# MorganGrundy/MosaicMagnifique

Hardware: NVIDIA B200
Metric: pixel-diffs/sec (higher is better)
Workload: dtype f32

## Files before the change

mosaicmagnifique_b200/csrc/diff_kernels.cu:

```cuda
#include <cuda_runtime.h>
#include <stdint.h>
#include <stdlib.h>

#include <algorithm>
#include <cub/device/device_scan.cuh>

#include "colour_math.cuh"
#include "kernels.h"

namespace mm {

__device__ __forceinline__ uint32_t smem_u32(const void *p) { return (uint32_t)__cvta_generic_to_shared(p); }

__device__ __forceinline__ void mbar_init(uint64_t *bar, uint32_t count)
{
    asm volatile("mbarrier.init.shared::cta.b64 [%0], %1;" ::"r"(smem_u32(bar)), "r"(count));
}
__device__ __forceinline__ void mbar_expect_tx(uint64_t *bar, uint32_t bytes)
{
    asm volatile("mbarrier.arrive.expect_tx.shared::cta.b64 _, [%0], %1;" ::"r"(smem_u32(bar)), "r"(bytes) : "memory");
}
__device__ __forceinline__ void mbar_arrive(uint64_t *bar)
{
    asm volatile("mbarrier.arrive.shared::cta.b64 _, [%0];" ::"r"(smem_u32(bar)) : "memory");
// ... 2 lines not shown
{
    asm volatile(
        "{\n"
        ".reg .pred p;\n"
        "WAIT_%=:\n"
        "mbarrier.try_wait.parity.shared::cta.b64 p, [%0], %1;\n"
        "@p bra DONE_%=;\n"
        "bra WAIT_%=;\n"
        "DONE_%=:\n"
        "}\n" ::"r"(smem_u32(bar)),
        "r"(parity)
        : "memory");
}
__device__ __forceinline__ void bulk_g2s(void *dst, const void *src, uint32_t bytes, uint64_t *bar)
{
    asm volatile("cp.async.bulk.shared::cluster.global.mbarrier::complete_tx::bytes [%0], [%1], %2, [%3];" ::"r"(
                     smem_u32(dst)),
                 "l"(src), "r"(bytes), "r"(smem_u32(bar))
                 : "memory");
}

#ifndef MM_PIXEL_UNROLL
#define MM_PIXEL_UNROLL 1
#endif
constexpr int kPixelUnroll = MM_PIXEL_UNROLL;
constexpr int kStages = MM_STAGES;
constexpr int kConsumerWarps = MM_TCB;
constexpr int kThreads = (kConsumerWarps + 1) * 32;
constexpr uint32_t kLibBlockBytes = MM_TNB * MM_KP * 16;
constexpr uint32_t kCellBlockBytes = MM_TCB * MM_KP * 20;
constexpr uint32_t kStageBytes = kLibBlockBytes + kCellBlockBytes;

template <int DIFF>
__device__ __forceinline__ void consume_ring(const unsigned char *smem, uint64_t *full_bar, uint64_t *empty_bar, int nk, int warp,
                                             int lane, float (&acc)[MM_TNB])
{
#pragma unroll
    for (int i = 0; i < MM_TNB; ++i)
        acc[i] = 0.0f;

    for (int k = 0; k < nk; ++k) {
        const int s = k % kStages;
        mbar_wait(&full_bar[s], (k / kStages) & 1);
        if (MM_STRESS_SKEW)
            __nanosleep((unsigned)((warp * 97 + k * 29 + blockIdx.x * 7) % 400));
        const float4 *lib_s = reinterpret_cast<const float4 *>(smem + (size_t)s * kStageBytes);
        const float4 *cell_s = reinterpret_cast<const float4 *>(smem + (size_t)s * kStageBytes + kLibBlockBytes) + warp * MM_KP;
        const float *w_s = reinterpret_cast<const float *>(smem + (size_t)s * kStageBytes + kLibBlockBytes + MM_TCB * MM_KP * 16) + warp * MM_KP;
#pragma unroll kPixelUnroll
        for (int j = 0; j < MM_KP / 32; ++j) {
            const int p = j * 32 + lane;
            const float4 c = cell_s[p];
            const float w = w_s[p];
            if (DIFF == MM_DIFF_CIEDE2000) {
#pragma unroll
                for (int i = 0; i < MM_TNB / 2; ++i) {
                    const float4 la = lib_s[(i * 2 + 0) * MM_KP + p];
                    const float4 lb = lib_s[(i * 2 + 1) * MM_KP + p];
                    const mm_f2 d = mm_ciede2000_stored_v<mm_f2>(c.x, c.y, c.z, c.w, mm_f2{la.x, la.y}, mm_f2{la.z, la.w},
                                                               mm_f2{lb.x, lb.y}, mm_f2{lb.z, lb.w});
                    const mm_f2 a2 = v_fma(mm_f2{w, w}, d, mm_f2{acc[2 * i], acc[2 * i + 1]});
                    acc[2 * i] = a2.x;
                    acc[2 * i + 1] = a2.y;
                }
            } else {
#pragma unroll
                for (int i = 0; i < MM_TNB; ++i) {
                    const float4 l = lib_s[i * MM_KP + p];
                    acc[i] = fmaf(w, mm_euclid(c.x, c.y, c.z, l.x, l.y, l.z), acc[i]);
                }
            }
        }
        __syncwarp();
        if (lane == 0)
            mbar_arrive(&empty_bar[s]);
    }
}

template <int DIFF>
__global__ void __launch_bounds__(kThreads, MM_MIN_CTAS)
diff_sum_kernel(const unsigned char *__restrict__ cells, const unsigned char *__restrict__ lib, float *__restrict__ D,
                unsigned long long *__restrict__ best_key, int n_chunks, int n_lib, int n_lib_pad, int n_cells,
                int n_cell_tiles, int n_lib_tiles, const int *__restrict__ cancel, unsigned long long *__restrict__ progress,
                int nk, int sb_a, int sb_b)
{
    extern __shared__ __align__(128) unsigned char smem[];
    __shared__ uint64_t full_bar[kStages];
    __shared__ uint64_t empty_bar[kStages];
    __shared__ int s_cancelled;

    const int warp = threadIdx.x >> 5, lane = threadIdx.x & 31;
    int cell_tile, lib_tile;
    {
        const unsigned id = blockIdx.x;
        const unsigned col_all = (unsigned)sb_a * (unsigned)n_lib_tiles;
        const unsigned cb = id / col_all;
        const unsigned r = id - cb * col_all;
        const int cw = min(sb_a, n_cell_tiles - (int)cb * sb_a);
        const unsigned band_ctas = (unsigned)cw * (unsigned)sb_b;
        const unsigned band = r / band_ctas;
        const unsigned r2 = r - band * band_ctas;
        cell_tile = (int)cb * sb_a + (int)(r2 % cw);
        lib_tile = (int)band * sb_b + (int)(r2 / cw);
    }

// ... 68 lines not shown
    if (e != cudaSuccess)
        return e;
    const unsigned grid = (unsigned)n_cell_tiles * (unsigned)n_lib_tiles;
    diff_sum_kernel<DIFF><<<grid, kThreads, smem, stream>>>((const unsigned char *)cells, (const unsigned char *)lib, D, best_key, n_chunks,
                                                            n_lib, n_lib_tiles * MM_TNB, n_cells, n_cell_tiles, n_lib_tiles, cancel,
                                                            progress, n_chunks, raster.sb_a, raster.sb_b);
    return cudaGetLastError();
}

cudaError_t launch_diff_sum(int diff_type, const void *cells, const void *lib, float *D, unsigned long long *best_key,
                            int n_cell_tiles, int n_lib_tiles, int n_chunks, int n_lib, int n_cells, cudaStream_t stream,
                            const int *cancel, unsigned long long *progress)
{
    if (n_cell_tiles <= 0 || n_lib_tiles <= 0 || n_chunks <= 0)
        return cudaSuccess;
    if (diff_type != MM_DIFF_CIEDE2000)
        return cudaErrorInvalidValue;
    auto env = [](const char *name) -> int {
        const char *v = getenv(name);
        return v ? atoi(v) : 0;
    };
    Raster r{std::min(kSuperTiles, n_cell_tiles), std::min(kSuperTiles, n_lib_tiles)};
    if (env("MM_SB_A") > 0)
        r.sb_a = std::min(env("MM_SB_A"), n_cell_tiles);
    if (env("MM_SB_B") > 0)
        r.sb_b = std::min(env("MM_SB_B"), n_lib_tiles);
    return launch<MM_DIFF_CIEDE2000>(cells, lib, D, best_key, n_cell_tiles, n_lib_tiles, n_chunks, n_lib, n_cells, stream, cancel, progress,
                                     r);
}


__global__ void __launch_bounds__(kThreads, MM_MIN_CTAS)
diff_rows_kernel(const unsigned char *__restrict__ cells, const unsigned char *__restrict__ lib, float *__restrict__ D, int n_chunks,
                 int nk, int n_lib_pad, int n_lib_tiles, RowList rows, const int *__restrict__ perm, const int *cancel,
                 unsigned long long *__restrict__ progress)
{
    extern __shared__ __align__(128) unsigned char smem[];
    __shared__ uint64_t full_bar[kStages];
    __shared__ uint64_t empty_bar[kStages];
    __shared__ int s_cancelled, s_cell[kConsumerWarps], s_lib_tile, s_n_rows;

    const int warp = threadIdx.x >> 5, lane = threadIdx.x & 31;
    if (threadIdx.x == 0) {
        const int cancelled = cancel ? load_cancel_flag(cancel) : 0;
        int lo = 0, hi = rows.n_buckets;
        while (hi - lo > 1) {
            const int mid = (lo + hi) >> 1;
            if (rows.groups[mid] <= (int)blockIdx.x)
                lo = mid;
            else
                hi = mid;
        }
        const int g = (int)blockIdx.x - rows.groups[lo];
        const int n_in = min(kConsumerWarps, rows.count[lo] - g * kConsumerWarps);
        const int *list = rows.cells + (size_t)lo * rows.col_cells + g * kConsumerWarps;
        for (int w = 0; w < kConsumerWarps; ++w)
            s_cell[w] = list[w < n_in ? w : 0];
        s_lib_tile = lo % n_lib_tiles;
        s_n_rows = n_in;
        for (int s = 0; s < kStages; ++s) {
            mbar_init(&full_bar[s], 1);
            mbar_init(&empty_bar[s], kConsumerWarps);
        }
        asm volatile("fence.mbarrier_init.release.cluster;" ::: "memory");
        s_cancelled = cancelled;
    }
    __syncthreads();
    if (s_cancelled)
        return;
    const int lib_tile = s_lib_tile;

    if (warp == kConsumerWarps) {
        if (lane == 0) {
            const unsigned char *lib_src = lib + (size_t)lib_tile * n_chunks * kLibBlockBytes;
            constexpr uint32_t kSlice = MM_KP * 16, kWSlice = MM_KP * 4;
            for (int k = 0; k < nk; ++k) {
                const int s = k % kStages;
                if (k >= kStages)
                    mbar_wait(&empty_bar[s], ((k / kStages) - 1) & 1);
                unsigned char *dst = smem + (size_t)s * kStageBytes;
                if (MM_STRESS_SKEW)
                    __nanosleep((unsigned)((k * 131 + blockIdx.x * 17) % 300));
                mbar_expect_tx(&full_bar[s], kLibBlockBytes + kConsumerWarps * (kSlice + kWSlice));
                bulk_g2s(dst, lib_src + (size_t)k * kLibBlockBytes, kLibBlockBytes, &full_bar[s]);
                for (int w = 0; w < kConsumerWarps; ++w) {
                    const int c = s_cell[w];
                    const unsigned char *blk = cells + ((size_t)(c / MM_TCB) * n_chunks + k) * kCellBlockBytes;
                    const int slot = c % MM_TCB;
                    bulk_g2s(dst + kLibBlockBytes + w * kSlice, blk + slot * kSlice, kSlice, &full_bar[s]);
                    bulk_g2s(dst + kLibBlockBytes + MM_TCB * kSlice + w * kWSlice, blk + MM_TCB * kSlice + slot * kWSlice, kWSlice,
                             &full_bar[s]);
                }
            }
        }
        return;
    }

    float acc[MM_TNB];
    consume_ring<MM_DIFF_CIEDE2000>(smem, full_bar, empty_bar, nk, warp, lane, acc);
#pragma unroll
    for (int i = 0; i < MM_TNB; ++i) {
        float v = acc[i];
#pragma unroll
        for (int o = 16; o > 0; o >>= 1)
            v += __shfl_xor_sync(0xffffffffu, v, o);
        acc[i] = v;
    }
    if (warp < s_n_rows && lane < MM_TNB) {
        float v = 0.0f;
#pragma unroll
        for (int i = 0; i < MM_TNB; ++i)
            v = (lane == i) ? acc[i] : v;
        float *d = D + (size_t)s_cell[warp] * n_lib_pad + perm[lib_tile * MM_TNB + lane];
        *d += v;
    }
    if (progress && threadIdx.x == 0)
        atomicAdd(progress, (unsigned long long)s_n_rows);
}

cudaError_t launch_diff_rows(const void *cells, const void *lib, float *D, int n_groups, int n_lib_tiles, int n_chunks, int k0, int nk,
                             RowList rows, const int *perm, cudaStream_t stream, const int *cancel, unsigned long long *progress)
{
    if (n_groups <= 0 || nk <= 0)
        return cudaSuccess;
    const size_t smem = (size_t)kStages * kStageBytes;
    cudaError_t e = cudaFuncSetAttribute(diff_rows_kernel, cudaFuncAttributeMaxDynamicSharedMemorySize, (int)smem);
    if (e != cudaSuccess)
        return e;
    diff_rows_kernel<<<(unsigned)n_groups, kThreads, smem, stream>>>(
        (const unsigned char *)cells + (size_t)k0 * kCellBlockBytes, (const unsigned char *)lib + (size_t)k0 * kLibBlockBytes, D, n_chunks, nk,
        n_lib_tiles * MM_TNB, n_lib_tiles, rows, perm, cancel, progress);
    return cudaGetLastError();
}

__global__ void __launch_bounds__(1024)
list_rows_kernel(float *__restrict__ D, int n_lib_pad, int n_lib, int n_rows, int n_lib_tiles, uint8_t *__restrict__ state, int want,
                 const float *__restrict__ T, const int *__restrict__ perm, int segs_left, RowList rows,
                 int *__restrict__ group_count, unsigned long long *__restrict__ listed, unsigned long long *__restrict__ progress)
{
    __shared__ int warp_sum[32];
    const int lib_tile = blockIdx.x, col = blockIdx.y;
    const int b = col * n_lib_tiles + lib_tile;
    const int cell = col * rows.col_cells + threadIdx.x;
    bool on = false;
    if (threadIdx.x < rows.col_cells && cell < n_rows) {
        uint8_t *st = state ? state + (size_t)cell * n_lib_tiles + lib_tile : nullptr;
        on = !st || *st == want;
        if (on && T) {
            const float t = T[cell];
            float *row = D + (size_t)cell * n_lib_pad;
            bool alive = false;
            for (int i = 0; i < MM_TNB; ++i) {
                const int j = perm[lib_tile * MM_TNB + i];
                alive = alive || (j < n_lib && row[j] <= t);
            }
            if (!alive) {
                for (int i = 0; i < MM_TNB; ++i)
                    row[perm[lib_tile * MM_TNB + i]] = __int_as_float(0x7f800000);
                *st = kRowDead;
                if (progress)
                    atomicAdd(progress, (unsigned long long)segs_left);
                on = false;
            }
        }
    }
    const int lane = threadIdx.x & 31, warp = threadIdx.x >> 5;
    const unsigned ballot = __ballot_sync(0xffffffffu, on);
    if (lane == 0)
        warp_sum[warp] = __popc(ballot);
    __syncthreads();
    int before = 0, total = 0;
    for (int w = 0; w < (int)(blockDim.x >> 5); ++w) {
        before += w < warp ? warp_sum[w] : 0;
        total += warp_sum[w];
    }
    if (on)
        rows.cells[(size_t)b * rows.col_cells + before + __popc(ballot & ((1u << lane) - 1u))] = cell;
    if (threadIdx.x == 0) {
        rows.count[b] = total;
        group_count[b] = (total + MM_TCB - 1) / MM_TCB;
        if (total)
            atomicAdd(listed, (unsigned long long)total);
    }
}

size_t list_rows_scratch_bytes(int n_buckets)
{
    size_t temp = 0;
    cub::DeviceScan::ExclusiveSum(nullptr, temp, (const int *)nullptr, (int *)nullptr, n_buckets + 1);
    return ((size_t)(n_buckets + 1) * sizeof(int) + 255 & ~(size_t)255) + temp;
}

cudaError_t launch_list_rows(float *D, int n_lib_pad, int n_lib, int n_rows, int n_lib_tiles, uint8_t *state, int want, const float *T,
                             const int *perm, int segs_left, RowList rows, void *scratch, size_t scratch_bytes,
                             unsigned long long *listed, unsigned long long *progress, cudaStream_t stream)
{
    const int n_cols = (n_rows + rows.col_cells - 1) / rows.col_cells;
    if (n_cols <= 0 || n_lib_tiles <= 0)
        return cudaSuccess;
    if (rows.col_cells > 1024 || rows.col_cells % 32 || rows.n_buckets != n_cols * n_lib_tiles)
        return cudaErrorInvalidValue;
    int *group_count = (int *)scratch;
    const size_t head = (size_t)(rows.n_buckets + 1) * sizeof(int) + 255 & ~(size_t)255;
    cudaError_t e = cudaMemsetAsync(group_count + rows.n_buckets, 0, sizeof(int), stream);
    if (e != cudaSuccess)
        return e;
    list_rows_kernel<<<dim3((unsigned)n_lib_tiles, (unsigned)n_cols), rows.col_cells, 0, stream>>>(
        D, n_lib_pad, n_lib, n_rows, n_lib_tiles, state, want, T, perm, segs_left, rows, group_count, listed, progress);
    if ((e = cudaGetLastError()) != cudaSuccess)
        return e;
    size_t temp = scratch_bytes - head;
    return cub::DeviceScan::ExclusiveSum((unsigned char *)scratch + head, temp, group_count, rows.groups, rows.n_buckets + 1, stream);
}

}
```

mosaicmagnifique_b200/csrc/generator.cu:

```cuda
#include <cuda_runtime.h>
#include <math.h>
#include <stdio.h>
#include <string.h>

#include <algorithm>
#include <atomic>
#include <chrono>
#include <string>
#include <thread>
#include <vector>

#include "../../include/mosaic_b200.h"
#include "host_model.h"
#include "kernels.h"

extern "C" const int16_t mm_lab_lut_s16[];

namespace {

using namespace mm;

struct Fail {
    int code;
    std::string msg;
// ... 27 lines not shown
    void release()
    {
        if (p)
            cudaFreeAsync(p, stream);
        p = nullptr;
        bytes = cap = 0;
    }
    template <typename T>
    T *as() const { return reinterpret_cast<T *>(p); }
    ~DevBuf() { release(); }
    DevBuf() = default;
    DevBuf(const DevBuf &) = delete;
    DevBuf &operator=(const DevBuf &) = delete;
    DevBuf(DevBuf &&o) noexcept : p(o.p), bytes(o.bytes), cap(o.cap), stream(o.stream)
    {
        o.p = nullptr;
        o.bytes = o.cap = 0;
    }
    DevBuf &operator=(DevBuf &&o) noexcept
    {
        if (this != &o) {
            release();
            p = o.p;
            bytes = o.bytes;
            cap = o.cap;
            stream = o.stream;
            o.p = nullptr;
            o.bytes = o.cap = 0;
        }
        return *this;
    }
};

constexpr int kPruneSegments = 8;
constexpr int kColumnCells = 256;

struct Workspace {
    DevBuf main_f32, main_var_u8, lib_small, lib_work, lib_half;
    DevBuf pix_list, masks4, descs, cells_packed, lib_packed, best_key;
    DevBuf grid, pos, next, prog, counts;
    DevBuf tab_start, tab_si, tab_alpha;
    DevBuf perm, inv_perm, order_scratch, row_cells, row_count, row_groups, list_scratch, row_state, listed, prune_score, prune_idx,
        threshold;
    DevBuf prefix_score, prefix_idx;
};

struct StepPlan {
    int rows = 0, cols = 0;
    int S = 0, ds = 0, k = 1;
    int n_active = 0, n_chunks = 0;
    std::vector<int> cell_pos;
    std::vector<int> next_x;
    std::vector<int> row_first;
    int64_t cell_begin = 0, cell_end = 0;
    int64_t per_rank = 0;
    double pixel_diffs = 0, pixel_diffs_nominal = 0;
};

struct StepOut {
    DevBuf D;
    DevBuf cand;
    DevBuf margins;
    bool have_D = false, have_margins = false;
    int cand_k = 0;
};

struct Handles {
    cudaStream_t stream = nullptr;
    cudaStream_t poll_stream = nullptr;
    int *h_cancel = nullptr;
    int *d_cancel = nullptr;
    unsigned long long *h_progress = nullptr;

    Handles() = default;
    Handles(const Handles &) = delete;
    Handles &operator=(const Handles &) = delete;
// ... 655 lines not shown
    w.n_rows_local = (int)(w.n_local * V);
    w.n_cell_tiles = (w.n_rows_local + tg.tcb - 1) / tg.tcb;
    w.n_rows_pad = w.n_cell_tiles * tg.tcb;
    d.descs.alloc(std::max<size_t>(descs.size(), 1) * sizeof(CellDesc), st);
    CU(cudaMemcpyAsync(d.descs.p, descs.data(), descs.size() * sizeof(CellDesc), cudaMemcpyHostToDevice, st));
    tm.h2d_bytes += (double)(descs.size() * sizeof(CellDesc));
    d.cells_packed.alloc((size_t)std::max(w.n_cell_tiles, 1) * p.n_chunks * tg.cell_block, st);
    AreaTab cell_tab{nullptr, nullptr, nullptr};
    if (p.k == 0)
        cell_tab = upload_area_table(g, p.S, p.ds, tm);
    CU(launch_extract_cells(d.main_f32.as<float>(), g->img_rows, g->img_cols, d.descs.as<CellDesc>(), w.n_rows_local, p.S, p.ds, p.k,
                            cell_tab, d.masks4.as<uint8_t>(), d.pix_list.as<int>(), p.n_active, p.n_chunks, d.cells_packed.p, r.layout,
                            st));
    tm.kernel_launches++;
}

void plan_step(const G *g, const Run &r, size_t s, StepWork &w)
{
    const StepPlan &p = g->plans[s];
    const int64_t N = r.N;
    w.need_D = !r.fused_argmin || g->keep_D;
    const int64_t rr = g->repeat_range;
    const int64_t n_win = 2 * rr * rr + 2 * rr;
    const int64_t n_excl = r.capped ? r.O * exhausted_bound(g, s) : 0;
    w.k_need = r.candidates_only ? ((r.penalise || r.capped) ? std::min<int64_t>(N, r.O * n_win + n_excl + 1) : 1)
                                 : std::min<int64_t>(N, r.O * n_win + n_excl + 1 + (g->report_margins ? 1 : 0));
    w.via_topk = r.candidates_only || ((r.penalise || r.capped) && w.k_need * 4 <= N);
    w.M = (int)std::min<int64_t>(N, w.k_need + w.k_need / 4 + 8);
    w.prune = r.row_passes && w.via_topk && r.V == 1 && !g->keep_D && w.k_need * 4 <= N && w.M <= 4096 && w.n_rows_local > 0;
    w.n_segs = 1;
    w.seg_chunks = p.n_chunks;
    if (r.row_passes) {
        const char *ev = getenv("MM_SPLITK");
        const int want = ev && atoi(ev) > 0 ? atoi(ev) : kPruneSegments;
        w.seg_chunks = (p.n_chunks + std::min(want, p.n_chunks) - 1) / std::min(want, p.n_chunks);
        w.n_segs = (p.n_chunks + w.seg_chunks - 1) / w.seg_chunks;
        if (const char *ea = getenv("MM_SB_A"))
            w.col_cells = std::max(32, std::min(1024, atoi(ea) * MM_TCB / 32 * 32));
    }
    w.prog_total = r.row_passes ? (unsigned long long)std::max(w.n_rows_local, 1) * r.n_lib_tiles * w.n_segs
                                : (unsigned long long)std::max(w.n_cell_tiles, 1) * r.n_lib_tiles;
}

double difference_sums(G *g, const Run &r, size_t s, const StepWork &w, Progress &prog, mosaic_timings &tm)
{
    cudaStream_t st = g->stream;
    const StepPlan &p = g->plans[s];
    Workspace &d = g->ws;
    StepOut &o = g->out[s];
    DevBuf &D = o.D;
    if (w.need_D) {
        D.alloc((size_t)std::max(w.n_rows_pad, 1) * r.n_lib_pad * sizeof(float), st);
        o.have_D = true;
    }
    if (r.fused_argmin) {
        d.best_key.alloc((size_t)std::max(w.n_rows_pad, 1) * sizeof(unsigned long long), st);
        CU(launch_fill_u64(d.best_key.as<unsigned long long>(), (size_t)std::max(w.n_rows_pad, 1), ~0ull, st));
        tm.kernel_launches++;
    }
    prog.start_step(s, w.prog_total);
    if (!r.row_passes || w.n_rows_local == 0) {
        float *Dp = w.need_D ? D.as<float>() : nullptr;
        unsigned long long *keys = r.fused_argmin ? d.best_key.as<unsigned long long>() : nullptr;
        if (r.layout == kLayoutCiede)
            CU(launch_diff_sum(MM_DIFF_CIEDE2000, d.cells_packed.p, d.lib_packed.p, Dp, keys, w.n_cell_tiles, r.n_lib_tiles, p.n_chunks,
                               (int)r.N, w.n_rows_local, st, g->d_cancel, prog.d_done));
        else
            CU(launch_diff_euclid(d.cells_packed.p, d.lib_packed.p, Dp, keys, w.n_cell_tiles, r.n_lib_tiles, p.n_chunks, (int)r.N,
                                  w.n_rows_local, st, g->d_cancel, prog.d_done));
        tm.kernel_launches += w.n_cell_tiles > 0;
        return 1.0;
    }

    CU(cudaMemsetAsync(D.p, 0, D.bytes, st));
    const int n_cols = (w.n_rows_local + w.col_cells - 1) / w.col_cells;
    RowList rows{nullptr, nullptr, nullptr, n_cols * r.n_lib_tiles, w.col_cells};
    d.row_cells.alloc((size_t)rows.n_buckets * w.col_cells * sizeof(int), st);
    d.row_count.alloc((size_t)rows.n_buckets * sizeof(int), st);
    d.row_groups.alloc((size_t)(rows.n_buckets + 1) * sizeof(int), st);
    d.list_scratch.alloc(list_rows_scratch_bytes(rows.n_buckets), st);
    d.listed.alloc(sizeof(unsigned long long), st);
    rows.cells = d.row_cells.as<int>();
    rows.count = d.row_count.as<int>();
    rows.groups = d.row_groups.as<int>();
    const int *perm = d.perm.as<int>();
    uint8_t *state = nullptr;
    if (w.prune) {
        d.row_state.alloc((size_t)w.n_rows_local * r.n_lib_tiles, st);
        CU(cudaMemsetAsync(d.row_state.p, kRowActive, d.row_state.bytes, st));
        state = d.row_state.as<uint8_t>();
    }
    double units = 0;
    int n_groups = 0;
    auto list = [&](uint8_t *st8, int want, const float *T, int segs_left) {
        CU(cudaMemsetAsync(d.listed.p, 0, sizeof(unsigned long long), st));
        CU(launch_list_rows(D.as<float>(), r.n_lib_pad, (int)r.N, w.n_rows_local, r.n_lib_tiles, st8, want, T, perm, segs_left, rows,
                            d.list_scratch.p, d.list_scratch.bytes, d.listed.as<unsigned long long>(), prog.d_done, st));
        CU(cudaMemcpyAsync(g->h_progress + 1, rows.groups + rows.n_buckets, sizeof(int), cudaMemcpyDeviceToHost, st));
        CU(cudaMemcpyAsync(g->h_progress + 2, d.listed.p, sizeof(unsigned long long), cudaMemcpyDeviceToHost, st));
        tm.kernel_launches += 2;
        prog.wait();
        n_groups = (int)*reinterpret_cast<const int *>(g->h_progress + 1);
        return (double)g->h_progress[2];
    };
    auto pass = [&](int seg, double n_listed) {
        const int k0 = seg * w.seg_chunks, nk = std::min(p.n_chunks, k0 + w.seg_chunks) - k0;
        CU(launch_diff_rows(d.cells_packed.p, d.lib_packed.p, D.as<float>(), n_groups, r.n_lib_tiles, p.n_chunks, k0, nk, rows, perm, st,
                            g->d_cancel, prog.d_done));
        tm.kernel_launches += n_groups > 0;
        units += n_listed * nk;
    };
    double n_listed = list(nullptr, kRowActive, nullptr, 0);
    if (!w.prune) {
        for (int seg = 0; seg < w.n_segs; ++seg)
            pass(seg, n_listed);
    } else {
        pass(0, n_listed);
        d.prune_score.alloc((size_t)w.n_rows_local * w.M * sizeof(float), st);
        d.prune_idx.alloc((size_t)w.n_rows_local * w.M * sizeof(int), st);
        d.threshold.alloc((size_t)w.n_rows_local * sizeof(float), st);
        CU(launch_topk(D.as<float>(), r.n_lib_pad, (int)r.N, w.n_rows_local, w.M, d.prune_score.as<float>(), d.prune_idx.as<int>(), st));
        CU(launch_prune_threshold(D.as<float>(), r.n_lib_pad, d.prune_idx.as<int>(), w.n_rows_local, w.M, (int)w.k_need,
                                  d.inv_perm.as<int>(), r.n_lib_tiles, state, nullptr, true, st));
        tm.kernel_launches += 2;
        if (w.n_segs > 1) {
            n_listed = list(state, kRowComplete, nullptr, 0);
            for (int seg = 1; seg < w.n_segs; ++seg)
                pass(seg, n_listed);
        }
        CU(launch_prune_threshold(D.as<float>(), r.n_lib_pad, d.prune_idx.as<int>(), w.n_rows_local, w.M, (int)w.k_need,
                                  d.inv_perm.as<int>(), r.n_lib_tiles, state, d.threshold.as<float>(), false, st));
        tm.kernel_launches++;
        for (int seg = 1; seg < w.n_segs; ++seg) {
            n_listed = list(state, kRowActive, d.threshold.as<float>(), w.n_segs - seg);
            pass(seg, n_listed);
        }
    }
    return units / ((double)w.n_rows_local * r.n_lib_tiles * p.n_chunks);
}

struct Candidates {
    const float *scores = nullptr;
    const int *idx = nullptr;
    int M = 0, M_stride = 0;
    const float *pscores = nullptr;
    const int *pidx = nullptr;
    int k0 = 0, p_stride = 0;
    long long rows_per_block = 0, block_stride = 0;
};

template <typename Source>
void select_step(G *g, size_t s, const unsigned long long *keys, Source &&candidates, int max_uses, bool restart_used, float *margins,
                 PhaseClock *launch_clock, mosaic_timings &tm)
{
    const StepPlan &p = g->plans[s];
    GridStep &gs = g->grid[s];
    Workspace &w = g->ws;
    cudaStream_t st = g->stream;
    const int n_all = (int)p.cell_pos.size();
    w.grid.alloc(gs.v.size() * sizeof(long long), st);
    CU(cudaMemcpyAsync(w.grid.p, gs.v.data(), gs.v.size() * sizeof(long long), cudaMemcpyHostToDevice, st));
    w.pos.alloc(std::max<size_t>(p.cell_pos.size(), 1) * sizeof(int), st);
    CU(cudaMemcpyAsync(w.pos.p, p.cell_pos.data(), p.cell_pos.size() * sizeof(int), cudaMemcpyHostToDevice, st));
    tm.h2d_bytes += (double)(gs.v.size() * sizeof(long long) + p.cell_pos.size() * sizeof(int));
    if (keys) {
        CU(launch_keys_to_grid(keys, w.pos.as<int>(), w.grid.as<long long>(), n_all, nullptr, st));
    } else {
        w.next.alloc(std::max<size_t>(p.next_x.size(), 1) * sizeof(int), st);
        CU(cudaMemcpyAsync(w.next.p, p.next_x.data(), p.next_x.size() * sizeof(int), cudaMemcpyHostToDevice, st));
        w.prog.alloc((size_t)p.rows * sizeof(int), st);
        CU(cudaMemcpyAsync(w.prog.p, p.row_first.data(), (size_t)p.rows * sizeof(int), cudaMemcpyHostToDevice, st));
// ... 124 lines not shown
    if (!g->d_lut.p) {
        const std::vector<int16_t> lut4 = expand_lab_lut(mm_lab_lut_s16);
        g->d_lut.alloc(lut4.size() * sizeof(int16_t), st);
        CU(cudaMemcpyAsync(g->d_lut.p, lut4.data(), g->d_lut.bytes, cudaMemcpyHostToDevice, st));
        CU(cudaStreamSynchronize(st));
        tm.h2d_bytes += (double)g->d_lut.bytes;
    }

    clock.begin(kPre);
    main_to_working_space(g, r, tm);
    const LibSource lib = prepare_library(g, r, tm);
    clock.end();

    if (g->out.size() != n_steps) {
        g->out.clear();
        g->out.resize(n_steps);
    }
    for (StepOut &o : g->out) {
        o.have_D = o.have_margins = false;
        o.cand_k = 0;
    }
    if (candidates_only) {
        g->cand_max_uses = g->max_uses;
        g->cap_last_step = -1;
    }
    if (r.row_passes) {
        g->ws.perm.alloc((size_t)r.n_lib_pad * sizeof(int), st);
        g->ws.inv_perm.alloc((size_t)r.n_lib_pad * sizeof(int), st);
        g->ws.order_scratch.alloc(library_order_scratch_bytes(r.N), st);
        CU(launch_library_order(lib.oriented, g->lib_stored_size, r.N, r.n_lib_pad, g->ws.perm.as<int>(), g->ws.inv_perm.as<int>(),
                                g->ws.order_scratch.p, g->ws.order_scratch.bytes, st));
        tm.kernel_launches += 3;
    }
    Progress prog(g);
    for (size_t s = 0; s < n_steps; ++s) {
        prog.check_cancel();
        StepWork w;
        clock.begin(kPre);
        prepare_step(g, r, lib, s, w, tm);
        clock.end();
        plan_step(g, r, s, w);

        clock.begin(kDiff);
        const double evaluated = difference_sums(g, r, s, w, prog, tm);
        tm.evaluated_pixel_diffs += g->plans[s].pixel_diffs * evaluated;
        clock.end();
        if (g->progress_fn)
            prog.wait();

        clock.begin(kSel);
        select_phase(g, r, s, w, tm);
        clock.end();
        prog.end_step();
    }
    prog.finish();
    tm.preprocess_ms = clock.sum(kPre);
    tm.diff_ms = clock.sum(kDiff);
    tm.select_ms = clock.sum(kSel);
    tm.total_ms = std::chrono::duration<double, std::milli>(std::chrono::steady_clock::now() - t_host0).count();
}

}


extern "C" {

const char *mosaic_version(void) { return "mosaicmagnifique_b200 0.1 (sm_100a)"; }

int mosaic_create(int device, mosaic_generator **out)
{
    if (!out)
        return MOSAIC_ERR_INVALID_ARGUMENT;
    *out = nullptr;
    int count = 0;
    if (cudaGetDeviceCount(&count) != cudaSuccess || device < 0 || device >= count) {
        cudaGetLastError();
        return MOSAIC_ERR_CUDA;
    }
    mosaic_generator *g = new (std::nothrow) mosaic_generator();
    if (!g)
        return MOSAIC_ERR_OUT_OF_MEMORY;
    g->device = device;
    if (cudaSetDevice(device) != cudaSuccess || cudaStreamCreateWithFlags(&g->stream, cudaStreamNonBlocking) != cudaSuccess ||
        cudaStreamCreateWithFlags(&g->poll_stream, cudaStreamNonBlocking) != cudaSuccess ||
        cudaHostAlloc((void **)&g->h_cancel, sizeof(int), cudaHostAllocDefault) != cudaSuccess ||
        cudaMalloc((void **)&g->d_cancel, 256) != cudaSuccess || cudaMemset(g->d_cancel, 0, 256) != cudaSuccess ||
        cudaHostAlloc((void **)&g->h_progress, 4 * sizeof(unsigned long long), cudaHostAllocDefault) != cudaSuccess) {
        mosaic_destroy(g);
// ... 775 lines not shown
```

mosaicmagnifique_b200/csrc/kernels.h:

```cpp
#pragma once
#include <cuda_runtime.h>
#include <stdint.h>

#include <vector>

#define MM_DIFF_RGB_EUCLIDEAN 0
#define MM_DIFF_CIE76 1
#define MM_DIFF_CIEDE2000 2
#define MM_DIFF_EUCLID 0

#define MM_TCB 8
#define MM_TNB 8
#ifndef MM_KP
#define MM_KP 128
#endif
#ifndef MM_STAGES
#define MM_STAGES 3
#endif
#ifndef MM_ESTAGES
#define MM_ESTAGES 3
#endif
#ifndef MM_STRESS_SKEW
#define MM_STRESS_SKEW 0
#endif
// ... 22 lines not shown
{
    const unsigned band_ctas = (unsigned)n_ct * kSuperTiles;
    const unsigned band = id / band_ctas;
    const unsigned r = id - band * band_ctas;
    const int band_h = min(kSuperTiles, n_lt - (int)band * kSuperTiles);
    const unsigned col_ctas = (unsigned)kSuperTiles * band_h;
    const unsigned cb = r / col_ctas;
    const unsigned r2 = r - cb * col_ctas;
    const int cw = min(kSuperTiles, n_ct - (int)cb * kSuperTiles);
    cell_tile = (int)cb * kSuperTiles + (int)(r2 % cw);
    lib_tile = (int)band * kSuperTiles + (int)(r2 / cw);
}
#endif

enum PackLayout { kLayoutCiede = 0, kLayoutEuclid = 1 };
struct TileGeom {
    int tcb, tnb, kp;
    size_t cell_block, lib_block;
};
inline TileGeom tile_geom(PackLayout l)
{
    return l == kLayoutEuclid ? TileGeom{MM_ETC, MM_ETN, MM_EKP, (size_t)MM_EKP * 4 * MM_ETC * 4, (size_t)MM_EKP * 3 * MM_ETN * 4}
                              : TileGeom{MM_TCB, MM_TNB, MM_KP, (size_t)MM_TCB * MM_KP * 20, (size_t)MM_TNB * MM_KP * 16};
}

cudaError_t launch_diff_euclid(const void *cells, const void *lib, float *D, unsigned long long *best_key, int n_cell_tiles,
                               int n_lib_tiles, int n_chunks, int n_lib, int n_cells, cudaStream_t stream,
                               const int *cancel = nullptr, unsigned long long *progress = nullptr);

cudaError_t launch_diff_sum(int diff_type, const void *cells, const void *lib, float *D, unsigned long long *best_key,
                            int n_cell_tiles, int n_lib_tiles, int n_chunks, int n_lib, int n_cells, cudaStream_t stream,
                            const int *cancel = nullptr, unsigned long long *progress = nullptr);

struct RowList {
    int *cells;
    int *count;
    int *groups;
    int n_buckets, col_cells;
};
enum : uint8_t { kRowActive = 0, kRowComplete = 1, kRowDead = 2 };
cudaError_t launch_diff_rows(const void *cells, const void *lib, float *D, int n_groups, int n_lib_tiles, int n_chunks, int k0, int nk,
                             RowList rows, const int *perm, cudaStream_t stream, const int *cancel = nullptr,
                             unsigned long long *progress = nullptr);
size_t list_rows_scratch_bytes(int n_buckets);
cudaError_t launch_list_rows(float *D, int n_lib_pad, int n_lib, int n_rows, int n_lib_tiles, uint8_t *state, int want, const float *T,
                             const int *perm, int segs_left, RowList rows, void *scratch, size_t scratch_bytes,
                             unsigned long long *listed, unsigned long long *progress, cudaStream_t stream);

cudaError_t launch_to_working_space(const uint8_t *bgr, size_t row_stride, int rows, int cols, float *out, bool is_lab,
                                    const short4 *lab_lut, const int *c8, cudaStream_t stream);
constexpr size_t kLabLutEntries = 33 * 33 * 33;
inline std::vector<int16_t> expand_lab_lut(const int16_t *lut3)
{
    std::vector<int16_t> out(kLabLutEntries * 4, 0);
    for (size_t i = 0; i < kLabLutEntries; ++i)
        for (int c = 0; c < 3; ++c)
            out[i * 4 + c] = lut3[i * 3 + c];
    return out;
}
cudaError_t launch_hue_rotate(const uint8_t *in, uint8_t *out, int rows, int cols, float rot, cudaStream_t stream);
cudaError_t launch_area_u8(const uint8_t *src, uint8_t *dst, int64_t n, int src_size, int k, cudaStream_t stream);
cudaError_t launch_orient_library(const uint8_t *src, uint8_t *dst, int64_t n, int S, int flips, cudaStream_t stream);
cudaError_t launch_area_f32(const float *src, float *dst, int64_t n, int src_size, int k, cudaStream_t stream);
struct AreaTab {
    const int *start;
    const int *si;
    const float *alpha;
};
cudaError_t launch_area_general_u8(const uint8_t *src, uint8_t *dst, int64_t n, int src_size, int dst_size, AreaTab tab,
                                   cudaStream_t stream);
cudaError_t launch_area_general_f32(const float *src, float *dst, int64_t n, int src_size, int dst_size, AreaTab tab,
                                    cudaStream_t stream);
struct CubicTab {
    const int *idx;
    const int16_t *coef;
};
cudaError_t launch_cubic_u8(const uint8_t *src, int sh, int sw, int cn, uint8_t *dst, int dh, int dw, CubicTab xt, CubicTab yt,
                            cudaStream_t stream);
cudaError_t launch_pack_library(const float *lib, void *packed, int64_t n, int P, const int *pix_list, int n_active,
                                int n_chunks, int n_lib_tiles, PackLayout layout, cudaStream_t stream, const int *perm = nullptr);
// ... 71 lines not shown
```

Measured before the change: 437.4 billion.

## Make row-pass kernel persistent with atomic group queue and no host sync

Converts the diff_rows kernel from one CTA per group into a persistent grid sized by occupancy. The producer warp pulls group descriptors from a global atomic counter and signals consumers through a shared ring, so groups flow through the pipeline without refilling per CTA. It also removes the per-pass host round-trip that read group counts, computing group descriptors on device and accumulating evaluated units on device, read once at the end. Segment sizing changes to fixed chunk counts. The exchange is an extra describe kernel and an atomic per group, plus more complex termination and cancellation logic.

```diff
diff --git a/mosaicmagnifique_b200/csrc/diff_kernels.cu b/mosaicmagnifique_b200/csrc/diff_kernels.cu
--- a/mosaicmagnifique_b200/csrc/diff_kernels.cu
+++ b/mosaicmagnifique_b200/csrc/diff_kernels.cu
@@ -58,6 +58,38 @@
 constexpr uint32_t kStageBytes = kLibBlockBytes + kCellBlockBytes;
 
 template <int DIFF>
+__device__ __forceinline__ void consume_stage(const unsigned char *smem, int s, int warp, int lane, float (&acc)[MM_TNB])
+{
+    const float4 *lib_s = reinterpret_cast<const float4 *>(smem + (size_t)s * kStageBytes);
+    const float4 *cell_s = reinterpret_cast<const float4 *>(smem + (size_t)s * kStageBytes + kLibBlockBytes) + warp * MM_KP;
+    const float *w_s = reinterpret_cast<const float *>(smem + (size_t)s * kStageBytes + kLibBlockBytes + MM_TCB * MM_KP * 16) + warp * MM_KP;
+#pragma unroll kPixelUnroll
+    for (int j = 0; j < MM_KP / 32; ++j) {
+        const int p = j * 32 + lane;
+        const float4 c = cell_s[p];
+        const float w = w_s[p];
+        if (DIFF == MM_DIFF_CIEDE2000) {
+#pragma unroll
+            for (int i = 0; i < MM_TNB / 2; ++i) {
+                const float4 la = lib_s[(i * 2 + 0) * MM_KP + p];
+                const float4 lb = lib_s[(i * 2 + 1) * MM_KP + p];
+                const mm_f2 d = mm_ciede2000_stored_v<mm_f2>(c.x, c.y, c.z, c.w, mm_f2{la.x, la.y}, mm_f2{la.z, la.w},
+                                                           mm_f2{lb.x, lb.y}, mm_f2{lb.z, lb.w});
+                const mm_f2 a2 = v_fma(mm_f2{w, w}, d, mm_f2{acc[2 * i], acc[2 * i + 1]});
+                acc[2 * i] = a2.x;
+                acc[2 * i + 1] = a2.y;
+            }
+        } else {
+#pragma unroll
+            for (int i = 0; i < MM_TNB; ++i) {
+                const float4 l = lib_s[i * MM_KP + p];
+                acc[i] = fmaf(w, mm_euclid(c.x, c.y, c.z, l.x, l.y, l.z), acc[i]);
+            }
+        }
+    }
+}
+
+template <int DIFF>
 __device__ __forceinline__ void consume_ring(const unsigned char *smem, uint64_t *full_bar, uint64_t *empty_bar, int nk, int warp,
                                              int lane, float (&acc)[MM_TNB])
 {
@@ -70,33 +102,7 @@
         mbar_wait(&full_bar[s], (k / kStages) & 1);
         if (MM_STRESS_SKEW)
             __nanosleep((unsigned)((warp * 97 + k * 29 + blockIdx.x * 7) % 400));
-        const float4 *lib_s = reinterpret_cast<const float4 *>(smem + (size_t)s * kStageBytes);
-        const float4 *cell_s = reinterpret_cast<const float4 *>(smem + (size_t)s * kStageBytes + kLibBlockBytes) + warp * MM_KP;
-        const float *w_s = reinterpret_cast<const float *>(smem + (size_t)s * kStageBytes + kLibBlockBytes + MM_TCB * MM_KP * 16) + warp * MM_KP;
-#pragma unroll kPixelUnroll
-        for (int j = 0; j < MM_KP / 32; ++j) {
-            const int p = j * 32 + lane;
-            const float4 c = cell_s[p];
-            const float w = w_s[p];
-            if (DIFF == MM_DIFF_CIEDE2000) {
-#pragma unroll
-                for (int i = 0; i < MM_TNB / 2; ++i) {
-                    const float4 la = lib_s[(i * 2 + 0) * MM_KP + p];
-                    const float4 lb = lib_s[(i * 2 + 1) * MM_KP + p];
-                    const mm_f2 d = mm_ciede2000_stored_v<mm_f2>(c.x, c.y, c.z, c.w, mm_f2{la.x, la.y}, mm_f2{la.z, la.w},
-                                                               mm_f2{lb.x, lb.y}, mm_f2{lb.z, lb.w});
-                    const mm_f2 a2 = v_fma(mm_f2{w, w}, d, mm_f2{acc[2 * i], acc[2 * i + 1]});
-                    acc[2 * i] = a2.x;
-                    acc[2 * i + 1] = a2.y;
-                }
-            } else {
-#pragma unroll
-                for (int i = 0; i < MM_TNB; ++i) {
-                    const float4 l = lib_s[i * MM_KP + p];
-                    acc[i] = fmaf(w, mm_euclid(c.x, c.y, c.z, l.x, l.y, l.z), acc[i]);
-                }
-            }
-        }
+        consume_stage<DIFF>(smem, s, warp, lane, acc);
         __syncwarp();
         if (lane == 0)
             mbar_arrive(&empty_bar[s]);
@@ -231,32 +237,17 @@
 
 __global__ void __launch_bounds__(kThreads, MM_MIN_CTAS)
 diff_rows_kernel(const unsigned char *__restrict__ cells, const unsigned char *__restrict__ lib, float *__restrict__ D, int n_chunks,
-                 int nk, int n_lib_pad, int n_lib_tiles, RowList rows, const int *__restrict__ perm, const int *cancel,
+                 int nk, int n_lib_pad, RowList rows, const int *__restrict__ perm, const int *cancel,
                  unsigned long long *__restrict__ progress)
 {
     extern __shared__ __align__(128) unsigned char smem[];
     __shared__ uint64_t full_bar[kStages];
     __shared__ uint64_t empty_bar[kStages];
-    __shared__ int s_cancelled, s_cell[kConsumerWarps], s_lib_tile, s_n_rows;
+    __shared__ int s_cancelled, s_group[kStages];
 
     const int warp = threadIdx.x >> 5, lane = threadIdx.x & 31;
     if (threadIdx.x == 0) {
         const int cancelled = cancel ? load_cancel_flag(cancel) : 0;
-        int lo = 0, hi = rows.n_buckets;
-        while (hi - lo > 1) {
-            const int mid = (lo + hi) >> 1;
-            if (rows.groups[mid] <= (int)blockIdx.x)
-                lo = mid;
-            else
-                hi = mid;
-        }
-        const int g = (int)blockIdx.x - rows.groups[lo];
-        const int n_in = min(kConsumerWarps, rows.count[lo] - g * kConsumerWarps);
-        const int *list = rows.cells + (size_t)lo * rows.col_cells + g * kConsumerWarps;
-        for (int w = 0; w < kConsumerWarps; ++w)
-            s_cell[w] = list[w < n_in ? w : 0];
-        s_lib_tile = lo % n_lib_tiles;
-        s_n_rows = n_in;
         for (int s = 0; s < kStages; ++s) {
             mbar_init(&full_bar[s], 1);
             mbar_init(&empty_bar[s], kConsumerWarps);
@@ -267,75 +258,121 @@
     __syncthreads();
     if (s_cancelled)
         return;
-    const int lib_tile = s_lib_tile;
 
     if (warp == kConsumerWarps) {
         if (lane == 0) {
-            const unsigned char *lib_src = lib + (size_t)lib_tile * n_chunks * kLibBlockBytes;
             constexpr uint32_t kSlice = MM_KP * 16, kWSlice = MM_KP * 4;
-            for (int k = 0; k < nk; ++k) {
-                const int s = k % kStages;
-                if (k >= kStages)
-                    mbar_wait(&empty_bar[s], ((k / kStages) - 1) & 1);
-                unsigned char *dst = smem + (size_t)s * kStageBytes;
-                if (MM_STRESS_SKEW)
-                    __nanosleep((unsigned)((k * 131 + blockIdx.x * 17) % 300));
-                mbar_expect_tx(&full_bar[s], kLibBlockBytes + kConsumerWarps * (kSlice + kWSlice));
-                bulk_g2s(dst, lib_src + (size_t)k * kLibBlockBytes, kLibBlockBytes, &full_bar[s]);
-                for (int w = 0; w < kConsumerWarps; ++w) {
-                    const int c = s_cell[w];
-                    const unsigned char *blk = cells + ((size_t)(c / MM_TCB) * n_chunks + k) * kCellBlockBytes;
-                    const int slot = c % MM_TCB;
-                    bulk_g2s(dst + kLibBlockBytes + w * kSlice, blk + slot * kSlice, kSlice, &full_bar[s]);
-                    bulk_g2s(dst + kLibBlockBytes + MM_TCB * kSlice + w * kWSlice, blk + MM_TCB * kSlice + slot * kWSlice, kWSlice,
-                             &full_bar[s]);
+            const int n_groups = rows.groups[rows.n_buckets];
+            for (int t = 0;;) {
+                const int cancelled = t > 0 && cancel ? load_cancel_flag(cancel) : 0;
+                const int g = atomicAdd(rows.next, 1);
+                const bool stop = g >= n_groups || cancelled;
+                int s = t % kStages;
+                if (t >= kStages)
+                    mbar_wait(&empty_bar[s], ((t / kStages) - 1) & 1);
+                *(volatile int *)&s_group[s] = stop ? -1 : g;
+                if (stop) {
+                    mbar_arrive(&full_bar[s]);
+                    return;
                 }
+                const GroupDesc &gd = rows.desc[g];
+                int cell[kConsumerWarps];
+#pragma unroll
+                for (int w = 0; w < kConsumerWarps; ++w)
+                    cell[w] = gd.cell[w];
+                const unsigned char *lib_src = lib + (size_t)gd.lib_tile * n_chunks * kLibBlockBytes;
+                for (int k = 0; k < nk; ++k, ++t, s = t % kStages) {
+                    if (k > 0 && t >= kStages)
+                        mbar_wait(&empty_bar[s], ((t / kStages) - 1) & 1);
+                    unsigned char *dst = smem + (size_t)s * kStageBytes;
+                    if (MM_STRESS_SKEW)
+                        __nanosleep((unsigned)((t * 131 + blockIdx.x * 17) % 300));
+                    mbar_expect_tx(&full_bar[s], kLibBlockBytes + kConsumerWarps * (kSlice + kWSlice));
+                    bulk_g2s(dst, lib_src + (size_t)k * kLibBlockBytes, kLibBlockBytes, &full_bar[s]);
+#pragma unroll
+                    for (int w = 0; w < kConsumerWarps; ++w) {
+                        const int c = cell[w];
+                        const unsigned char *blk = cells + ((size_t)(c / MM_TCB) * n_chunks + k) * kCellBlockBytes;
+                        const int slot = c % MM_TCB;
+                        bulk_g2s(dst + kLibBlockBytes + w * kSlice, blk + slot * kSlice, kSlice, &full_bar[s]);
+                        bulk_g2s(dst + kLibBlockBytes + MM_TCB * kSlice + w * kWSlice, blk + MM_TCB * kSlice + slot * kWSlice, kWSlice,
+                                 &full_bar[s]);
+                    }
+                }
             }
         }
         return;
     }
 
     float acc[MM_TNB];
-    consume_ring<MM_DIFF_CIEDE2000>(smem, full_bar, empty_bar, nk, warp, lane, acc);
-#pragma unroll
-    for (int i = 0; i < MM_TNB; ++i) {
-        float v = acc[i];
-#pragma unroll
-        for (int o = 16; o > 0; o >>= 1)
-            v += __shfl_xor_sync(0xffffffffu, v, o);
-        acc[i] = v;
-    }
-    if (warp < s_n_rows && lane < MM_TNB) {
-        float v = 0.0f;
+#pragma unroll
+    for (int i = 0; i < MM_TNB; ++i)
+        acc[i] = 0.0f;
+    for (int t = 0, g = 0, k = 0;; ++t) {
+        const int s = t % kStages;
+        mbar_wait(&full_bar[s], (t / kStages) & 1);
+        if (k == 0 && (g = *(volatile int *)&s_group[s]) < 0)
+            return;
+        if (MM_STRESS_SKEW)
+            __nanosleep((unsigned)((warp * 97 + t * 29 + blockIdx.x * 7) % 400));
+        consume_stage<MM_DIFF_CIEDE2000>(smem, s, warp, lane, acc);
+        __syncwarp();
+        if (lane == 0)
+            mbar_arrive(&empty_bar[s]);
+        if (++k < nk)
+            continue;
+#pragma unroll
+        for (int i = 0; i < MM_TNB; ++i) {
+            float v = acc[i];
+#pragma unroll
+            for (int o = 16; o > 0; o >>= 1)
+                v += __shfl_xor_sync(0xffffffffu, v, o);
+            acc[i] = v;
+        }
+        const GroupDesc *gd = rows.desc + g;
+        const int n_rows = gd->n_rows;
+        if (warp < n_rows && lane < MM_TNB) {
+            float v = 0.0f;
+#pragma unroll
+            for (int i = 0; i < MM_TNB; ++i)
+                v = (lane == i) ? acc[i] : v;
+            D[(size_t)gd->cell[warp] * n_lib_pad + perm[gd->lib_tile * MM_TNB + lane]] += v;
+        }
+        if (progress && threadIdx.x == 0)
+            atomicAdd(progress, (unsigned long long)n_rows);
+        k = 0;
 #pragma unroll
         for (int i = 0; i < MM_TNB; ++i)
-            v = (lane == i) ? acc[i] : v;
-        float *d = D + (size_t)s_cell[warp] * n_lib_pad + perm[lib_tile * MM_TNB + lane];
-        *d += v;
-    }
-    if (progress && threadIdx.x == 0)
-        atomicAdd(progress, (unsigned long long)s_n_rows);
-}
-
-cudaError_t launch_diff_rows(const void *cells, const void *lib, float *D, int n_groups, int n_lib_tiles, int n_chunks, int k0, int nk,
-                             RowList rows, const int *perm, cudaStream_t stream, const int *cancel, unsigned long long *progress)
-{
-    if (n_groups <= 0 || nk <= 0)
+            acc[i] = 0.0f;
+    }
+}
+
+cudaError_t launch_diff_rows(const void *cells, const void *lib, float *D, int n_lib_tiles, int n_chunks, int k0, int nk, RowList rows,
+                             const int *perm, cudaStream_t stream, const int *cancel, unsigned long long *progress)
+{
+    if (rows.n_buckets <= 0 || nk <= 0)
         return cudaSuccess;
     const size_t smem = (size_t)kStages * kStageBytes;
     cudaError_t e = cudaFuncSetAttribute(diff_rows_kernel, cudaFuncAttributeMaxDynamicSharedMemorySize, (int)smem);
     if (e != cudaSuccess)
         return e;
-    diff_rows_kernel<<<(unsigned)n_groups, kThreads, smem, stream>>>(
+    if ((e = cudaMemsetAsync(rows.next, 0, sizeof(int), stream)) != cudaSuccess)
+        return e;
+    int dev = 0, n_sm = 0, per_sm = 0;
+    if ((e = cudaGetDevice(&dev)) != cudaSuccess || (e = cudaDeviceGetAttribute(&n_sm, cudaDevAttrMultiProcessorCount, dev)) != cudaSuccess ||
+        (e = cudaOccupancyMaxActiveBlocksPerMultiprocessor(&per_sm, diff_rows_kernel, kThreads, smem)) != cudaSuccess)
+        return e;
+    diff_rows_kernel<<<(unsigned)(n_sm * std::max(per_sm, 1)), kThreads, smem, stream>>>(
         (const unsigned char *)cells + (size_t)k0 * kCellBlockBytes, (const unsigned char *)lib + (size_t)k0 * kLibBlockBytes, D, n_chunks, nk,
-        n_lib_tiles * MM_TNB, n_lib_tiles, rows, perm, cancel, progress);
+        n_lib_tiles * MM_TNB, rows, perm, cancel, progress);
     return cudaGetLastError();
 }
 
 __global__ void __launch_bounds__(1024)
 list_rows_kernel(float *__restrict__ D, int n_lib_pad, int n_lib, int n_rows, int n_lib_tiles, uint8_t *__restrict__ state, int want,
                  const float *__restrict__ T, const int *__restrict__ perm, int segs_left, RowList rows,
-                 int *__restrict__ group_count, unsigned long long *__restrict__ listed, unsigned long long *__restrict__ progress)
+                 int *__restrict__ group_count, int unit_chunks, unsigned long long *__restrict__ units,
+                 unsigned long long *__restrict__ progress)
 {
     __shared__ int warp_sum[32];
     const int lib_tile = blockIdx.x, col = blockIdx.y;
@@ -379,8 +416,24 @@
         rows.count[b] = total;
         group_count[b] = (total + MM_TCB - 1) / MM_TCB;
         if (total)
-            atomicAdd(listed, (unsigned long long)total);
-    }
+            atomicAdd(units, (unsigned long long)total * unit_chunks);
+    }
+}
+
+__global__ void describe_groups_kernel(RowList rows, int n_lib_tiles)
+{
+    const int b = blockIdx.x, g = threadIdx.x;
+    const int n = rows.count[b] - g * MM_TCB;
+    if (n <= 0)
+        return;
+    const int *list = rows.cells + (size_t)b * rows.col_cells + g * MM_TCB;
+    GroupDesc d;
+    d.lib_tile = b % n_lib_tiles;
+    d.n_rows = min(MM_TCB, n);
+#pragma unroll
+    for (int w = 0; w < MM_TCB; ++w)
+        d.cell[w] = list[w < d.n_rows ? w : 0];
+    rows.desc[rows.groups[b] + g] = d;
 }
 
 size_t list_rows_scratch_bytes(int n_buckets)
@@ -391,8 +444,8 @@
 }
 
 cudaError_t launch_list_rows(float *D, int n_lib_pad, int n_lib, int n_rows, int n_lib_tiles, uint8_t *state, int want, const float *T,
-                             const int *perm, int segs_left, RowList rows, void *scratch, size_t scratch_bytes,
-                             unsigned long long *listed, unsigned long long *progress, cudaStream_t stream)
+                             const int *perm, int segs_left, RowList rows, void *scratch, size_t scratch_bytes, int unit_chunks,
+                             unsigned long long *units, unsigned long long *progress, cudaStream_t stream)
 {
     const int n_cols = (n_rows + rows.col_cells - 1) / rows.col_cells;
     if (n_cols <= 0 || n_lib_tiles <= 0)
@@ -405,11 +458,15 @@
     if (e != cudaSuccess)
         return e;
     list_rows_kernel<<<dim3((unsigned)n_lib_tiles, (unsigned)n_cols), rows.col_cells, 0, stream>>>(
-        D, n_lib_pad, n_lib, n_rows, n_lib_tiles, state, want, T, perm, segs_left, rows, group_count, listed, progress);
+        D, n_lib_pad, n_lib, n_rows, n_lib_tiles, state, want, T, perm, segs_left, rows, group_count, unit_chunks, units, progress);
     if ((e = cudaGetLastError()) != cudaSuccess)
         return e;
     size_t temp = scratch_bytes - head;
-    return cub::DeviceScan::ExclusiveSum((unsigned char *)scratch + head, temp, group_count, rows.groups, rows.n_buckets + 1, stream);
-}
-
-}
+    if ((e = cub::DeviceScan::ExclusiveSum((unsigned char *)scratch + head, temp, group_count, rows.groups, rows.n_buckets + 1, stream)) !=
+        cudaSuccess)
+        return e;
+    describe_groups_kernel<<<(unsigned)rows.n_buckets, rows.col_cells / MM_TCB, 0, stream>>>(rows, n_lib_tiles);
+    return cudaGetLastError();
+}
+
+}
diff --git a/mosaicmagnifique_b200/csrc/generator.cu b/mosaicmagnifique_b200/csrc/generator.cu
--- a/mosaicmagnifique_b200/csrc/generator.cu
+++ b/mosaicmagnifique_b200/csrc/generator.cu
@@ -83,7 +83,8 @@
     }
 };
 
-constexpr int kPruneSegments = 8;
+constexpr int kSegChunks = 4;
+constexpr int kMinSegments = 8;
 constexpr int kColumnCells = 256;
 
 struct Workspace {
@@ -91,8 +92,8 @@
     DevBuf pix_list, masks4, descs, cells_packed, lib_packed, best_key;
     DevBuf grid, pos, next, prog, counts;
     DevBuf tab_start, tab_si, tab_alpha;
-    DevBuf perm, inv_perm, order_scratch, row_cells, row_count, row_groups, list_scratch, row_state, listed, prune_score, prune_idx,
-        threshold;
+    DevBuf perm, inv_perm, order_scratch, row_cells, row_count, row_groups, row_desc, row_next, list_scratch, row_state, units, prune_score,
+        prune_idx, threshold;
     DevBuf prefix_score, prefix_idx;
 };
 
@@ -814,8 +815,10 @@
     w.seg_chunks = p.n_chunks;
     if (r.row_passes) {
         const char *ev = getenv("MM_SPLITK");
-        const int want = ev && atoi(ev) > 0 ? atoi(ev) : kPruneSegments;
-        w.seg_chunks = (p.n_chunks + std::min(want, p.n_chunks) - 1) / std::min(want, p.n_chunks);
+        if (ev && atoi(ev) > 0)
+            w.seg_chunks = (p.n_chunks + std::min(atoi(ev), p.n_chunks) - 1) / std::min(atoi(ev), p.n_chunks);
+        else
+            w.seg_chunks = std::min(kSegChunks, (p.n_chunks + kMinSegments - 1) / kMinSegments);
         w.n_segs = (p.n_chunks + w.seg_chunks - 1) / w.seg_chunks;
         if (const char *ea = getenv("MM_SB_A"))
             w.col_cells = std::max(32, std::min(1024, atoi(ea) * MM_TCB / 32 * 32));
@@ -824,7 +827,7 @@
                                 : (unsigned long long)std::max(w.n_cell_tiles, 1) * r.n_lib_tiles;
 }
 
-double difference_sums(G *g, const Run &r, size_t s, const StepWork &w, Progress &prog, mosaic_timings &tm)
+void difference_sums(G *g, const Run &r, size_t s, const StepWork &w, Progress &prog, mosaic_timings &tm)
 {
     cudaStream_t st = g->stream;
     const StepPlan &p = g->plans[s];
@@ -851,20 +854,23 @@
             CU(launch_diff_euclid(d.cells_packed.p, d.lib_packed.p, Dp, keys, w.n_cell_tiles, r.n_lib_tiles, p.n_chunks, (int)r.N,
                                   w.n_rows_local, st, g->d_cancel, prog.d_done));
         tm.kernel_launches += w.n_cell_tiles > 0;
-        return 1.0;
+        return;
     }
 
     CU(cudaMemsetAsync(D.p, 0, D.bytes, st));
     const int n_cols = (w.n_rows_local + w.col_cells - 1) / w.col_cells;
-    RowList rows{nullptr, nullptr, nullptr, n_cols * r.n_lib_tiles, w.col_cells};
+    RowList rows{nullptr, nullptr, nullptr, nullptr, nullptr, n_cols * r.n_lib_tiles, w.col_cells};
     d.row_cells.alloc((size_t)rows.n_buckets * w.col_cells * sizeof(int), st);
     d.row_count.alloc((size_t)rows.n_buckets * sizeof(int), st);
     d.row_groups.alloc((size_t)(rows.n_buckets + 1) * sizeof(int), st);
+    d.row_desc.alloc((size_t)rows.n_buckets * (w.col_cells / MM_TCB) * sizeof(GroupDesc), st);
     d.list_scratch.alloc(list_rows_scratch_bytes(rows.n_buckets), st);
-    d.listed.alloc(sizeof(unsigned long long), st);
     rows.cells = d.row_cells.as<int>();
     rows.count = d.row_count.as<int>();
     rows.groups = d.row_groups.as<int>();
+    rows.desc = d.row_desc.as<GroupDesc>();
+    d.row_next.alloc(sizeof(int), st);
+    rows.next = d.row_next.as<int>();
     const int *perm = d.perm.as<int>();
     uint8_t *state = nullptr;
     if (w.prune) {
@@ -872,53 +878,46 @@
         CU(cudaMemsetAsync(d.row_state.p, kRowActive, d.row_state.bytes, st));
         state = d.row_state.as<uint8_t>();
     }
-    double units = 0;
-    int n_groups = 0;
-    auto list = [&](uint8_t *st8, int want, const float *T, int segs_left) {
-        CU(cudaMemsetAsync(d.listed.p, 0, sizeof(unsigned long long), st));
+    unsigned long long *units = d.units.as<unsigned long long>() + s;
+    auto seg_k0 = [&](int seg) { return seg * w.seg_chunks; };
+    auto seg_nk = [&](int seg) { return std::min(p.n_chunks, seg_k0(seg) + w.seg_chunks) - seg_k0(seg); };
+    auto list = [&](uint8_t *st8, int want, const float *T, int segs_left, int unit_chunks) {
         CU(launch_list_rows(D.as<float>(), r.n_lib_pad, (int)r.N, w.n_rows_local, r.n_lib_tiles, st8, want, T, perm, segs_left, rows,
-                            d.list_scratch.p, d.list_scratch.bytes, d.listed.as<unsigned long long>(), prog.d_done, st));
-        CU(cudaMemcpyAsync(g->h_progress + 1, rows.groups + rows.n_buckets, sizeof(int), cudaMemcpyDeviceToHost, st));
-        CU(cudaMemcpyAsync(g->h_progress + 2, d.listed.p, sizeof(unsigned long long), cudaMemcpyDeviceToHost, st));
-        tm.kernel_launches += 2;
-        prog.wait();
-        n_groups = (int)*reinterpret_cast<const int *>(g->h_progress + 1);
-        return (double)g->h_progress[2];
+                            d.list_scratch.p, d.list_scratch.bytes, unit_chunks, units, prog.d_done, st));
+        tm.kernel_launches += 3;
     };
-    auto pass = [&](int seg, double n_listed) {
-        const int k0 = seg * w.seg_chunks, nk = std::min(p.n_chunks, k0 + w.seg_chunks) - k0;
-        CU(launch_diff_rows(d.cells_packed.p, d.lib_packed.p, D.as<float>(), n_groups, r.n_lib_tiles, p.n_chunks, k0, nk, rows, perm, st,
-                            g->d_cancel, prog.d_done));
-        tm.kernel_launches += n_groups > 0;
-        units += n_listed * nk;
+    auto pass = [&](int seg) {
+        CU(launch_diff_rows(d.cells_packed.p, d.lib_packed.p, D.as<float>(), r.n_lib_tiles, p.n_chunks, seg_k0(seg), seg_nk(seg), rows, perm,
+                            st, g->d_cancel, prog.d_done));
+        tm.kernel_launches++;
     };
-    double n_listed = list(nullptr, kRowActive, nullptr, 0);
     if (!w.prune) {
+        list(nullptr, kRowActive, nullptr, 0, p.n_chunks);
         for (int seg = 0; seg < w.n_segs; ++seg)
-            pass(seg, n_listed);
-    } else {
-        pass(0, n_listed);
-        d.prune_score.alloc((size_t)w.n_rows_local * w.M * sizeof(float), st);
-        d.prune_idx.alloc((size_t)w.n_rows_local * w.M * sizeof(int), st);
-        d.threshold.alloc((size_t)w.n_rows_local * sizeof(float), st);
-        CU(launch_topk(D.as<float>(), r.n_lib_pad, (int)r.N, w.n_rows_local, w.M, d.prune_score.as<float>(), d.prune_idx.as<int>(), st));
-        CU(launch_prune_threshold(D.as<float>(), r.n_lib_pad, d.prune_idx.as<int>(), w.n_rows_local, w.M, (int)w.k_need,
-                                  d.inv_perm.as<int>(), r.n_lib_tiles, state, nullptr, true, st));
-        tm.kernel_launches += 2;
-        if (w.n_segs > 1) {
-            n_listed = list(state, kRowComplete, nullptr, 0);
-            for (int seg = 1; seg < w.n_segs; ++seg)
-                pass(seg, n_listed);
-        }
-        CU(launch_prune_threshold(D.as<float>(), r.n_lib_pad, d.prune_idx.as<int>(), w.n_rows_local, w.M, (int)w.k_need,
-                                  d.inv_perm.as<int>(), r.n_lib_tiles, state, d.threshold.as<float>(), false, st));
-        tm.kernel_launches++;
-        for (int seg = 1; seg < w.n_segs; ++seg) {
-            n_listed = list(state, kRowActive, d.threshold.as<float>(), w.n_segs - seg);
-            pass(seg, n_listed);
-        }
-    }
-    return units / ((double)w.n_rows_local * r.n_lib_tiles * p.n_chunks);
+            pass(seg);
+        return;
+    }
+    list(nullptr, kRowActive, nullptr, 0, seg_nk(0));
+    pass(0);
+    d.prune_score.alloc((size_t)w.n_rows_local * w.M * sizeof(float), st);
+    d.prune_idx.alloc((size_t)w.n_rows_local * w.M * sizeof(int), st);
+    d.threshold.alloc((size_t)w.n_rows_local * sizeof(float), st);
+    CU(launch_topk(D.as<float>(), r.n_lib_pad, (int)r.N, w.n_rows_local, w.M, d.prune_score.as<float>(), d.prune_idx.as<int>(), st));
+    CU(launch_prune_threshold(D.as<float>(), r.n_lib_pad, d.prune_idx.as<int>(), w.n_rows_local, w.M, (int)w.k_need,
+                              d.inv_perm.as<int>(), r.n_lib_tiles, state, nullptr, true, st));
+    tm.kernel_launches += 2;
+    if (w.n_segs > 1) {
+        list(state, kRowComplete, nullptr, 0, p.n_chunks - seg_nk(0));
+        for (int seg = 1; seg < w.n_segs; ++seg)
+            pass(seg);
+    }
+    CU(launch_prune_threshold(D.as<float>(), r.n_lib_pad, d.prune_idx.as<int>(), w.n_rows_local, w.M, (int)w.k_need,
+                              d.inv_perm.as<int>(), r.n_lib_tiles, state, d.threshold.as<float>(), false, st));
+    tm.kernel_launches++;
+    for (int seg = 1; seg < w.n_segs; ++seg) {
+        list(state, kRowActive, d.threshold.as<float>(), w.n_segs - seg, seg_nk(seg));
+        pass(seg);
+    }
 }
 
 struct Candidates {
@@ -1109,6 +1108,11 @@
                                 g->ws.order_scratch.p, g->ws.order_scratch.bytes, st));
         tm.kernel_launches += 3;
     }
+    std::vector<double> units_complete(n_steps, 0.0);
+    if (r.row_passes) {
+        g->ws.units.alloc(n_steps * sizeof(unsigned long long), st);
+        CU(cudaMemsetAsync(g->ws.units.p, 0, g->ws.units.bytes, st));
+    }
     Progress prog(g);
     for (size_t s = 0; s < n_steps; ++s) {
         prog.check_cancel();
@@ -1117,10 +1121,11 @@
         prepare_step(g, r, lib, s, w, tm);
         clock.end();
         plan_step(g, r, s, w);
+        if (r.row_passes && w.n_rows_local > 0)
+            units_complete[s] = (double)w.n_rows_local * r.n_lib_tiles * g->plans[s].n_chunks;
 
         clock.begin(kDiff);
-        const double evaluated = difference_sums(g, r, s, w, prog, tm);
-        tm.evaluated_pixel_diffs += g->plans[s].pixel_diffs * evaluated;
+        difference_sums(g, r, s, w, prog, tm);
         clock.end();
         if (g->progress_fn)
             prog.wait();
@@ -1131,6 +1136,13 @@
         prog.end_step();
     }
     prog.finish();
+    std::vector<unsigned long long> units(n_steps, 0);
+    if (r.row_passes) {
+        CU(cudaMemcpyAsync(units.data(), g->ws.units.p, n_steps * sizeof(unsigned long long), cudaMemcpyDeviceToHost, st));
+        CU(cudaStreamSynchronize(st));
+    }
+    for (size_t s = 0; s < n_steps; ++s)
+        tm.evaluated_pixel_diffs += g->plans[s].pixel_diffs * (units_complete[s] > 0 ? (double)units[s] / units_complete[s] : 1.0);
     tm.preprocess_ms = clock.sum(kPre);
     tm.diff_ms = clock.sum(kDiff);
     tm.select_ms = clock.sum(kSel);
diff --git a/mosaicmagnifique_b200/csrc/kernels.h b/mosaicmagnifique_b200/csrc/kernels.h
--- a/mosaicmagnifique_b200/csrc/kernels.h
+++ b/mosaicmagnifique_b200/csrc/kernels.h
@@ -78,20 +78,25 @@
                             int n_cell_tiles, int n_lib_tiles, int n_chunks, int n_lib, int n_cells, cudaStream_t stream,
                             const int *cancel = nullptr, unsigned long long *progress = nullptr);
 
+struct GroupDesc {
+    int lib_tile, n_rows;
+    int cell[MM_TCB];
+};
 struct RowList {
     int *cells;
     int *count;
     int *groups;
+    GroupDesc *desc;
+    int *next;
     int n_buckets, col_cells;
 };
 enum : uint8_t { kRowActive = 0, kRowComplete = 1, kRowDead = 2 };
-cudaError_t launch_diff_rows(const void *cells, const void *lib, float *D, int n_groups, int n_lib_tiles, int n_chunks, int k0, int nk,
-                             RowList rows, const int *perm, cudaStream_t stream, const int *cancel = nullptr,
-                             unsigned long long *progress = nullptr);
+cudaError_t launch_diff_rows(const void *cells, const void *lib, float *D, int n_lib_tiles, int n_chunks, int k0, int nk, RowList rows,
+                             const int *perm, cudaStream_t stream, const int *cancel = nullptr, unsigned long long *progress = nullptr);
 size_t list_rows_scratch_bytes(int n_buckets);
 cudaError_t launch_list_rows(float *D, int n_lib_pad, int n_lib, int n_rows, int n_lib_tiles, uint8_t *state, int want, const float *T,
-                             const int *perm, int segs_left, RowList rows, void *scratch, size_t scratch_bytes,
-                             unsigned long long *listed, unsigned long long *progress, cudaStream_t stream);
+                             const int *perm, int segs_left, RowList rows, void *scratch, size_t scratch_bytes, int unit_chunks,
+                             unsigned long long *units, unsigned long long *progress, cudaStream_t stream);
 
 cudaError_t launch_to_working_space(const uint8_t *bgr, size_t row_stride, int rows, int cols, float *out, bool is_lab,
                                     const short4 *lab_lut, const int *c8, cudaStream_t stream);
```

After: 444.6 billion, median of 6. 1.6% higher.
